# SerezD/gen_adversarial

Measured on AMD Instinct MI355X. Metric: purified images/sec (attack+encode+decode), higher is better.
Workload: dtype f32 storage; contractions as 3x bf16 MFMA (hi/lo split), fp32 accumulate; 1 GPU; configs[1]: NVAE purify + VGG-11, 64x64, PGD-Linf step (fwd + input-grad), bs 256 images/GPU x EoT 32 = 8192 defender rows per step, alphas ours_cosine_no_preprocessing_ids.yaml x0.7, assumed NVAE config (C=32, 3x8 groups, 20 latents); images_per_gpu=256, eot=32, rows_per_gpu=8192, chunk_rows=1024, streams=2, parallelism=image-sharded x1

## Files before the change

gen_adversarial_amd/csrc/conv_thin3.hip:

```cpp
#include "conv_split.h"
#include "conv_epilogue.h"

namespace ga {

constexpr int TK_TH = 8, TK_TW = 16;
constexpr int TK_PH = TK_TH + 2, TK_PW = TK_TW + 2, TK_P = TK_PH * TK_PW;
template <int CIN> struct thin_traits {
    static constexpr int KS = CIN / 16;
    static constexpr int Q = CIN / 4;
    static constexpr int QSH = CIN == 32 ? 3 : 4;
    static constexpr int LDH = CIN + 8;
    static constexpr int RS = CIN == 32 ? 768 : 1408;
    static constexpr int PLANE = TK_PH * RS;
    static constexpr int BFR = 9 * KS * 2 * 64 * 8;
    static constexpr int SLOTS = (TK_P * Q + 255) / 256;
    static constexpr int WGS_PER_CU = CIN == 32 ? 2 : 1;
    static constexpr size_t LDS = (size_t)(BFR + 2 * PLANE) * 2;
};

struct thin_geom { int H, W, tiles_x, tpi, ntiles, per; fastdiv fd_tpi, fd_tx; };

template <int CIN, int AFF, int ACT>
__global__ void __launch_bounds__(256, thin_traits<CIN>::WGS_PER_CU)
conv_thin3_kernel(const ga_conv_desc d, const thin_geom g, const int M) {
    using T = thin_traits<CIN>;
    constexpr int TK_C = CIN, TK_LDH = T::LDH, TK_RS = T::RS, TK_PLANE = T::PLANE, TK_BFR = T::BFR, TK_SLOTS = T::SLOTS, KS = T::KS;
    extern __shared__ __attribute__((aligned(16))) float smem[];
    __bf16* Bs = reinterpret_cast<__bf16*>(smem);
    __bf16* Ph = Bs + TK_BFR;
    __bf16* Pl = Ph + TK_PLANE;
    float* Cs = reinterpret_cast<float*>(Ph);

    const int tid = threadIdx.x, lane = tid & 63, wave = tid >> 6;
    const int c4 = tid & (T::Q - 1), lrow = lane & 31, lh = lane >> 5;
    const int nt = blockIdx.y, n0 = nt * 32;
    constexpr int INV = 0x7fffffff;
    const __amdgpu_buffer_rsrc_t rsrcX = __builtin_amdgcn_make_buffer_rsrc(const_cast<float*>(d.x), 0, d.x_bytes, 0x00020000);

    {
        const uintx4* wf = reinterpret_cast<const uintx4*>(d.w_frag) + (size_t)nt * (TK_BFR / 8);
#pragma unroll
        for (int i = 0; i < TK_BFR / 8 / 256; ++i) reinterpret_cast<uintx4*>(Bs)[tid + 256 * i] = wf[tid + 256 * i];
    }
    int slot_yx[TK_SLOTS], slot_lds[TK_SLOTS];
#pragma unroll
    for (int j = 0; j < TK_SLOTS; ++j) {
        const int pp = (tid + 256 * j) >> T::QSH;
        const int py = pp / TK_PW, px = pp - py * TK_PW;
        slot_yx[j] = pp < TK_P ? (py << 8) | px : -1;
        slot_lds[j] = py * TK_RS + px * TK_LDH + 4 * c4;
    }
    floatx4 rs = {1.f, 1.f, 1.f, 1.f}, rt = {0.f, 0.f, 0.f, 0.f};
    if (AFF == 1) {
        rs = *reinterpret_cast<const floatx4*>(d.pro_scale + 4 * c4);
        rt = *reinterpret_cast<const floatx4*>(d.pro_shift + 4 * c4);
    }
    const int o = wave * 32 + lrow;
    const __bf16* fa_h = Ph + (o >> 4) * TK_RS + (o & 15) * TK_LDH + 8 * lh;
    const __bf16* fa_l = fa_h + TK_PLANE;
    const __bf16* fb = Bs + lane * 8;

    const int t0 = blockIdx.x * g.per, t1 = min(g.ntiles, t0 + g.per);
    floatx4 rpat[TK_SLOTS], ps = rs, pt = rt;
    unsigned okmask = 0;
    int cur_n = 0, cur_y0 = 0, cur_x0 = 0;
    auto origin = [&](const int t, int& n, int& y0, int& x0) __attribute__((always_inline)) {
        n = fd_div(t, g.fd_tpi);
        const int rem = t - n * g.tpi, ty = fd_div(rem, g.fd_tx);
        y0 = ty * TK_TH;
        x0 = (rem - ty * g.tiles_x) * TK_TW;
    };
    auto issue = [&](const int t) __attribute__((always_inline)) {
        origin(t, cur_n, cur_y0, cur_x0);
        okmask = 0;
#pragma unroll
        for (int j = 0; j < TK_SLOTS; ++j) {
            const int y = cur_y0 - 1 + (slot_yx[j] >> 8), x = cur_x0 - 1 + (slot_yx[j] & 255);
            const bool ok = slot_yx[j] >= 0 && y >= 0 && y < g.H && x >= 0 && x < g.W;
            const int off = ok ? (((cur_n * g.H + y) * g.W + x) * d.ldx + 4 * c4) * 4 : INV;
            okmask |= (ok ? 1u : 0u) << j;
            rpat[j] = __builtin_bit_cast(floatx4, __builtin_amdgcn_raw_buffer_load_b128(rsrcX, off, 0, 0));
        }
        if (AFF == 2) {
            ps = *reinterpret_cast<const floatx4*>(d.pro_scale + (size_t)cur_n * TK_C + 4 * c4);
            pt = *reinterpret_cast<const floatx4*>(d.pro_shift + (size_t)cur_n * TK_C + 4 * c4);
        }
    };
    auto convert = [&]() __attribute__((always_inline)) {
        const floatx4 zero = {0.f, 0.f, 0.f, 0.f};
#pragma unroll
        for (int j = 0; j < TK_SLOTS; ++j) {
            floatx4 v = rpat[j];
            if (AFF == 1) v = pro_affine4(v, rs, rt, d.flags & GA_CONV_PRO_PRELU);
            if (AFF == 2) v = v * ps + pt;
            v = pro_act4<ACT>(v);
            if (AFF != 0) v = (okmask >> j) & 1u ? v : zero;
            bf16x4 hi, lo;
            split4(v, hi, lo);
            if (slot_yx[j] >= 0) {
                *reinterpret_cast<bf16x4*>(Ph + slot_lds[j]) = hi;
                *reinterpret_cast<bf16x4*>(Pl + slot_lds[j]) = lo;
            }
        }
    };

    if (t0 < t1) issue(t0);
    for (int t = t0; t < t1; ++t) {
        const int m_base = (cur_n * g.H + cur_y0) * g.W + cur_x0;
        convert();
        __syncthreads();
        if (t + 1 < t1) issue(t + 1);
        floatx16 acc[1][1];
#pragma unroll
        for (int r = 0; r < 16; ++r) acc[0][0][r] = 0.f;
#pragma unroll
        for (int ch = 0; ch < KS / 2; ++ch) {
#pragma unroll
            for (int tap = 0; tap < 9; ++tap) {
                const int tapoff = (tap / 3) * TK_RS + (tap % 3) * TK_LDH;
#pragma unroll
                for (int k2 = 0; k2 < 2; ++k2) {
                    const int ks = 2 * ch + k2;
                    const bf16x8 ah = *reinterpret_cast<const bf16x8*>(fa_h + tapoff + ks * 16);
                    const bf16x8 al = *reinterpret_cast<const bf16x8*>(fa_l + tapoff + ks * 16);
                    const bf16x8 bh = *reinterpret_cast<const bf16x8*>(fb + ((tap * KS + ks) * 2 + 0) * 512);
                    const bf16x8 bl = *reinterpret_cast<const bf16x8*>(fb + ((tap * KS + ks) * 2 + 1) * 512);
                    mfma3(acc[0][0], ah, al, bh, bl);
                }
            }
        }
        __syncthreads();
        conv_epilogue<4, 1, 1, 1>(d, acc, Cs, m_base, n0, M, 1, 1, 0, 4, g.W);
        __syncthreads();
    }
}

template <int CIN, int AFF, int ACT>
static void launch_thin_inst(const ga_conv_desc& d, hipStream_t stream, dim3 grid, const thin_geom& g, int M) {
    static dyn_lds_cache attr;
    const size_t lds = thin_traits<CIN>::LDS;
    (void)ensure_dyn_lds(attr, reinterpret_cast<const void*>(&conv_thin3_kernel<CIN, AFF, ACT>), lds);
    hipLaunchKernelGGL((conv_thin3_kernel<CIN, AFF, ACT>), grid, dim3(256), lds, stream, d, g, M);
}

int conv_thin3_supports(const ga_conv_desc& d) {
    if (d.KH != 3 || d.KW != 3 || d.sn != 1 || d.sd != 1 || d.pad != 1 || d.C2 != 0 || (d.C1 != 32 && d.C1 != 64)) return 0;
    if (d.Ho != d.Hi || d.Wo != d.Wi || d.Ho % TK_TH || d.Wo % TK_TW || d.Wo > 255 * TK_TW) return 0;
    return conv3_mode_supported(d);
}

template <int CIN>
static int thin_dispatch_c(const ga_conv_desc& d, hipStream_t stream, dim3 grid, const thin_geom& g, int M) {
#define GA_THIN(MODE, A, C, WIDE) case MODE: launch_thin_inst<CIN, A, C>(d, stream, grid, g, M); break;
    switch (conv_pro_mode(d)) {
        GA_CONV3_MODES(GA_THIN)
        default: return GA_E_UNSUPPORTED;
    }
#undef GA_THIN
    return check_launch();
}

int conv_thin3_dispatch(const ga_conv_desc& d, hipStream_t stream, int vec_out, int splits) {
    if (!vec_out || splits != 1 || !d.w_frag || !aligned16(d.w_frag) || !conv_thin3_supports(d)) return GA_E_UNSUPPORTED;
    const int M = d.N * d.Ho * d.Wo;
    thin_geom g;
    g.H = d.Ho; g.W = d.Wo;
    g.tiles_x = d.Wo / TK_TW;
    g.tpi = g.tiles_x * (d.Ho / TK_TH);
    g.ntiles = d.N * g.tpi;
    const int NT = (d.Cout + 31) / 32;
    int G = (d.C1 == 32 ? 512 : 256) / NT;
    if (G < 1) G = 1;
    if (G > g.ntiles) G = g.ntiles;
    g.per = (g.ntiles + G - 1) / G;
    G = (g.ntiles + g.per - 1) / g.per;
    g.fd_tpi = make_fastdiv(g.tpi);
    g.fd_tx = make_fastdiv(g.tiles_x);
    const dim3 grid(G, NT);
    return d.C1 == 32 ? thin_dispatch_c<32>(d, stream, grid, g, M) : thin_dispatch_c<64>(d, stream, grid, g, M);
}

}
```

Measured before the change: 6405 defender rows/s (rows = images x EoT-32).

## Compute two 32-wide output-channel blocks per workgroup in thin 3x3 conv

For 32-input-channel convs with 33-64 output channels, each workgroup now holds weights for both 32-channel output blocks and accumulates both from one staged input patch. The input tile is loaded and converted to hi/lo bf16 once instead of once per output block, removing redundant global reads and split work. In exchange, LDS and register use roughly double, occupancy drops to one workgroup per CU, and the grid halves (256 workgroups instead of 512 across two column blocks).

```diff
diff --git a/gen_adversarial_amd/csrc/conv_thin3.hip b/gen_adversarial_amd/csrc/conv_thin3.hip
--- a/gen_adversarial_amd/csrc/conv_thin3.hip
+++ b/gen_adversarial_amd/csrc/conv_thin3.hip
@@ -5,7 +5,7 @@
 
 constexpr int TK_TH = 8, TK_TW = 16;
 constexpr int TK_PH = TK_TH + 2, TK_PW = TK_TW + 2, TK_P = TK_PH * TK_PW;
-template <int CIN> struct thin_traits {
+template <int CIN, int NB = 1> struct thin_traits {
     static constexpr int KS = CIN / 16;
     static constexpr int Q = CIN / 4;
     static constexpr int QSH = CIN == 32 ? 3 : 4;
@@ -14,33 +14,38 @@
     static constexpr int PLANE = TK_PH * RS;
     static constexpr int BFR = 9 * KS * 2 * 64 * 8;
     static constexpr int SLOTS = (TK_P * Q + 255) / 256;
-    static constexpr int WGS_PER_CU = CIN == 32 ? 2 : 1;
-    static constexpr size_t LDS = (size_t)(BFR + 2 * PLANE) * 2;
+    static constexpr int WGS_PER_CU = (CIN == 32 && NB == 1) ? 2 : 1;
+    static constexpr int WTOT = NB * BFR;
+    static constexpr int STAGE = 128 * (32 * NB + 4) * 2;
+    static constexpr int WIN = 2 * PLANE > STAGE ? 2 * PLANE : STAGE;
+    static constexpr size_t LDS = (size_t)(WTOT + WIN) * 2;
+    static_assert(NB == 1 || (NB == 2 && CIN == 32), "two output blocks: 32 input channels only");
+    static_assert(LDS <= 160 * 1024, "LDS");
 };
 
 struct thin_geom { int H, W, tiles_x, tpi, ntiles, per; fastdiv fd_tpi, fd_tx; };
 
-template <int CIN, int AFF, int ACT>
-__global__ void __launch_bounds__(256, thin_traits<CIN>::WGS_PER_CU)
+template <int CIN, int AFF, int ACT, int NB = 1>
+__global__ void __launch_bounds__(256, (thin_traits<CIN, NB>::WGS_PER_CU))
 conv_thin3_kernel(const ga_conv_desc d, const thin_geom g, const int M) {
-    using T = thin_traits<CIN>;
+    using T = thin_traits<CIN, NB>;
     constexpr int TK_C = CIN, TK_LDH = T::LDH, TK_RS = T::RS, TK_PLANE = T::PLANE, TK_BFR = T::BFR, TK_SLOTS = T::SLOTS, KS = T::KS;
     extern __shared__ __attribute__((aligned(16))) float smem[];
     __bf16* Bs = reinterpret_cast<__bf16*>(smem);
-    __bf16* Ph = Bs + TK_BFR;
+    __bf16* Ph = Bs + T::WTOT;
     __bf16* Pl = Ph + TK_PLANE;
     float* Cs = reinterpret_cast<float*>(Ph);
 
     const int tid = threadIdx.x, lane = tid & 63, wave = tid >> 6;
     const int c4 = tid & (T::Q - 1), lrow = lane & 31, lh = lane >> 5;
-    const int nt = blockIdx.y, n0 = nt * 32;
+    const int nt = blockIdx.y, n0 = nt * 32 * NB;
     constexpr int INV = 0x7fffffff;
     const __amdgpu_buffer_rsrc_t rsrcX = __builtin_amdgcn_make_buffer_rsrc(const_cast<float*>(d.x), 0, d.x_bytes, 0x00020000);
 
     {
-        const uintx4* wf = reinterpret_cast<const uintx4*>(d.w_frag) + (size_t)nt * (TK_BFR / 8);
+        const uintx4* wf = reinterpret_cast<const uintx4*>(d.w_frag) + (size_t)nt * (T::WTOT / 8);
 #pragma unroll
-        for (int i = 0; i < TK_BFR / 8 / 256; ++i) reinterpret_cast<uintx4*>(Bs)[tid + 256 * i] = wf[tid + 256 * i];
+        for (int i = 0; i < T::WTOT / 8 / 256; ++i) reinterpret_cast<uintx4*>(Bs)[tid + 256 * i] = wf[tid + 256 * i];
     }
     int slot_yx[TK_SLOTS], slot_lds[TK_SLOTS];
 #pragma unroll
@@ -110,9 +115,11 @@
         convert();
         __syncthreads();
         if (t + 1 < t1) issue(t + 1);
-        floatx16 acc[1][1];
+        floatx16 acc[1][NB];
 #pragma unroll
-        for (int r = 0; r < 16; ++r) acc[0][0][r] = 0.f;
+        for (int b = 0; b < NB; ++b)
+#pragma unroll
+            for (int r = 0; r < 16; ++r) acc[0][b][r] = 0.f;
 #pragma unroll
         for (int ch = 0; ch < KS / 2; ++ch) {
 #pragma unroll
@@ -123,25 +130,30 @@
                     const int ks = 2 * ch + k2;
                     const bf16x8 ah = *reinterpret_cast<const bf16x8*>(fa_h + tapoff + ks * 16);
                     const bf16x8 al = *reinterpret_cast<const bf16x8*>(fa_l + tapoff + ks * 16);
-                    const bf16x8 bh = *reinterpret_cast<const bf16x8*>(fb + ((tap * KS + ks) * 2 + 0) * 512);
-                    const bf16x8 bl = *reinterpret_cast<const bf16x8*>(fb + ((tap * KS + ks) * 2 + 1) * 512);
-                    mfma3(acc[0][0], ah, al, bh, bl);
+#pragma unroll
+                    for (int b = 0; b < NB; ++b) {
+                        const bf16x8 bh = *reinterpret_cast<const bf16x8*>(fb + b * TK_BFR + ((tap * KS + ks) * 2 + 0) * 512);
+                        const bf16x8 bl = *reinterpret_cast<const bf16x8*>(fb + b * TK_BFR + ((tap * KS + ks) * 2 + 1) * 512);
+                        mfma3(acc[0][b], ah, al, bh, bl);
+                    }
                 }
             }
         }
         __syncthreads();
-        conv_epilogue<4, 1, 1, 1>(d, acc, Cs, m_base, n0, M, 1, 1, 0, 4, g.W);
+        conv_epilogue<4, 1, 1, NB>(d, acc, Cs, m_base, n0, M, 1, 1, 0, 4, g.W);
         __syncthreads();
     }
 }
 
-template <int CIN, int AFF, int ACT>
+template <int CIN, int AFF, int ACT, int NB>
 static void launch_thin_inst(const ga_conv_desc& d, hipStream_t stream, dim3 grid, const thin_geom& g, int M) {
     static dyn_lds_cache attr;
-    const size_t lds = thin_traits<CIN>::LDS;
-    (void)ensure_dyn_lds(attr, reinterpret_cast<const void*>(&conv_thin3_kernel<CIN, AFF, ACT>), lds);
-    hipLaunchKernelGGL((conv_thin3_kernel<CIN, AFF, ACT>), grid, dim3(256), lds, stream, d, g, M);
+    const size_t lds = thin_traits<CIN, NB>::LDS;
+    (void)ensure_dyn_lds(attr, reinterpret_cast<const void*>(&conv_thin3_kernel<CIN, AFF, ACT, NB>), lds);
+    hipLaunchKernelGGL((conv_thin3_kernel<CIN, AFF, ACT, NB>), grid, dim3(256), lds, stream, d, g, M);
 }
+
+static int thin_blocks(const ga_conv_desc& d) { return d.C1 == 32 && d.Cout > 32 && d.Cout <= 64 ? 2 : 1; }
 
 int conv_thin3_supports(const ga_conv_desc& d) {
     if (d.KH != 3 || d.KW != 3 || d.sn != 1 || d.sd != 1 || d.pad != 1 || d.C2 != 0 || (d.C1 != 32 && d.C1 != 64)) return 0;
@@ -149,9 +161,9 @@
     return conv3_mode_supported(d);
 }
 
-template <int CIN>
+template <int CIN, int NB = 1>
 static int thin_dispatch_c(const ga_conv_desc& d, hipStream_t stream, dim3 grid, const thin_geom& g, int M) {
-#define GA_THIN(MODE, A, C, WIDE) case MODE: launch_thin_inst<CIN, A, C>(d, stream, grid, g, M); break;
+#define GA_THIN(MODE, A, C, WIDE) case MODE: launch_thin_inst<CIN, A, C, NB>(d, stream, grid, g, M); break;
     switch (conv_pro_mode(d)) {
         GA_CONV3_MODES(GA_THIN)
         default: return GA_E_UNSUPPORTED;
@@ -168,8 +180,9 @@
     g.tiles_x = d.Wo / TK_TW;
     g.tpi = g.tiles_x * (d.Ho / TK_TH);
     g.ntiles = d.N * g.tpi;
-    const int NT = (d.Cout + 31) / 32;
-    int G = (d.C1 == 32 ? 512 : 256) / NT;
+    const int nb = thin_blocks(d);
+    const int NT = nb > 1 ? 1 : (d.Cout + 31) / 32;
+    int G = (d.C1 == 32 && nb == 1 ? 512 : 256) / NT;
     if (G < 1) G = 1;
     if (G > g.ntiles) G = g.ntiles;
     g.per = (g.ntiles + G - 1) / G;
@@ -177,6 +190,7 @@
     g.fd_tpi = make_fastdiv(g.tpi);
     g.fd_tx = make_fastdiv(g.tiles_x);
     const dim3 grid(G, NT);
+    if (nb == 2) return thin_dispatch_c<32, 2>(d, stream, grid, g, M);
     return d.C1 == 32 ? thin_dispatch_c<32>(d, stream, grid, g, M) : thin_dispatch_c<64>(d, stream, grid, g, M);
 }
 
```

New measurement: 6409 defender rows/s (rows = images x EoT-32) (median of 6 runs). No clear change (+0.1%).
